# gopi-erabati/Object-Pose-Estimation

Hardware: AMD Instinct MI355X
Metric: ICP iterations/sec (1M scene pts vs 100k model pts) at 1/2/4/8 GPU (higher is better)
Workload: dtype f32

## Files before the change

### object-pose-estimation_amd/csrc/api.hip

```cpp
#include <algorithm>
#include <cfloat>
#include <cmath>
#include <cstring>
#include <limits>
#include <numeric>

#include <chrono>
#include <thread>

#include "ope_internal.hpp"

namespace ope {

void launch_icp_accumulate(hipStream_t, int, int, bool, bool, const CloudView &, const BvhView &, const BvhView &,
                           const IcpState *, double *, int32_t *, float *, uint32_t *, uint32_t *, const uint32_t *,
                           uint32_t *, const uint32_t *, bool, int, double *, const uint32_t *, float *, const uint32_t *, hipEvent_t, hipEvent_t, bool,
                           uint32_t *, uint32_t, float4 *, uint32_t *, uint32_t *, uint32_t, uint32_t, float *);
void plan_heavy(hipStream_t, const uint32_t *, uint32_t, float, float, uint32_t, uint32_t *);
void plan_slots(hipStream_t, const uint32_t *, uint32_t, const uint32_t *, uint32_t *);
int icp_accumulate_blocks_per_cu(bool, bool, bool);
int icp_accumulate_cert_blocks_per_cu(bool, bool, bool);
int chunk_plan(hipStream_t, const uint32_t *, uint32_t *, const uint32_t *, uint32_t *, uint32_t, void *, size_t &);
void fill_iota(hipStream_t, uint32_t *, uint32_t);
hipError_t concat_device(hipStream_t, const CloudView &, const float *, const CloudView &, float *, float[3], float[3], const uint32_t *,
                         const uint32_t *, uint32_t *);
hipError_t build_bvh_device(hipStream_t, const float4 *, const float4 *, size_t, int, const float[3], const float[3], int *, float4 **,
                            float4 **, float4 **, float4 **, bool);
void launch_icp_accumulate_grid(hipStream_t, int, bool, const CloudView &, const BvhView &, const GridView &, const IcpState *, double *, int32_t *,
                                float *, uint32_t *, uint32_t *, const uint32_t *, unsigned char *, const uint32_t *, uint32_t *, const uint32_t *,
                                double *, hipEvent_t, hipEvent_t, bool, uint32_t *, uint32_t, uint32_t *, uint32_t, uint32_t, float4 *, uint32_t *, uint32_t *, float *);
int grid_plan(hipStream_t, bool, const unsigned char *, uint32_t, uint32_t *, uint32_t *, const uint32_t *, uint32_t *, uint32_t *, const uint32_t *,
              uint32_t *, uint32_t, uint32_t, float, float, void *, size_t);
// ... 13 lines not shown
void launch_lm_pos_to_orig(hipStream_t, const BvhView &, int32_t *, uint32_t);
void launch_nn_search(hipStream_t, const CloudView &, const BvhView &, const float *, int32_t *, float *);
void launch_knn_search(hipStream_t, const CloudView &, const BvhView &, const float *, int, int32_t *, float *);
void launch_fitness(hipStream_t, int, const CloudView &, const BvhView &, const float *, double, double *, const uint32_t *);
void launch_seed_hints(hipStream_t, const CloudView &, const BvhView &, const IcpState *, uint32_t *);
void launch_pairs_svd(hipStream_t, const float *, const float *, uint32_t, double *, int, float *);
int comm_allreduce_sums(ope_ctx *ctx, double *d_sums, int count);
bool comm_uses_p2p(const ope_ctx *ctx);
int comm_p2p_exchange_update(ope_ctx *ctx, IcpState *d_state, double *d_sums, int nsums);
int comm_p2p_exchange(ope_ctx *ctx, double *d_sums, int nsums);

static thread_local std::string g_global_err;

constexpr double kGridMaxTreeShare = 0.03, kGridMinTreeShare = 0.015;
constexpr size_t kGridMinQueries = 0;
constexpr float kHeavyLoadFactor = 1.5f;
constexpr float kHeavyMaxChunksPerWave = 1.8f;

int set_err(ope_ctx *ctx, int code, const std::string &msg) {
  if (ctx) ctx->err = msg;
  else g_global_err = msg;
  return code;
}

static inline bool finite3(const float *p) { return std::isfinite(p[0]) && std::isfinite(p[1]) && std::isfinite(p[2]); }

static void colmajor_to_rows(const float *T, float rows[12]) {
  for (int r = 0; r < 3; ++r)
    for (int c = 0; c < 4; ++c) rows[4 * r + c] = T[4 * c + r];
}

// ... 107 lines not shown
  }
  if (ctx->use_grid) {
    const ope_icp_params &p = ctx->run_params;
    const bool nrm = p.use_surface_normal_rej || p.use_self_occluded_rej || p.estimator == OPE_EST_POINT_TO_PLANE_LLS;
    const bool plan_step = !no_plan && nch > 1 && it_done >= 1 && plan_step_after(ctx, it_done);
    if (grid_probe_poll(ctx, it_done) < 0) {
      const int rcs = switch_kernel(ctx, false, it_done, nch);
      if (rcs != OPE_OK) return rcs;
      --ctx->acc_launches;
      return enqueue_accumulate(ctx, atomic_sums);
    }
    if (plan_step) {
      const bool repart = it_done <= 4 || it_done % kPlanPeriod == 0 || it_done == ctx->force_plan_at;
      if (grid_plan(ctx->stream, repart, ctx->d_qclass, (uint32_t)ctx->run_src->n_valid, ctx->d_qorder, ctx->d_work_counter + 8, cost_r,
                    ctx->d_chunk_keys, ctx->d_chunk_cost_sorted, ctx->d_chunk_ids, ctx->d_chunk_order, nch,
                    (uint32_t)ctx->acc_blocks * (kAccBlock / 64), -1.0f , kHeavyLoadFactor, ctx->d_part_tmp, ctx->part_tmp_bytes) != 0)
        return set_err(ctx, OPE_EHIP, "grid plan step failed");
      ctx->plan_valid = true;
      if (it_done == 1 || it_done >= 8) {
        const int rcp = grid_probe_issue(ctx);
        if (rcp != OPE_OK) return rcp;
      }
    }
    const bool timed = ctx->prof_enabled && ctx->prof_used < ctx->prof_events.size() / 2;
    const bool certify = ctx->cert_run && ctx->cert_seen;
    ctx->launch_blocks = certify ? std::min(ctx->acc_blocks, ctx->acc_blocks_cert) : ctx->acc_blocks;
    ++ctx->kernel_launches[OPE_KERNEL_GRID];
    launch_icp_accumulate_grid(ctx->stream, ctx->launch_blocks, nrm, ctx->run_src->view(), ctx->run_tgt->view(), ctx->run_tgt->grid, ctx->d_state,
                               ctx->d_partials, ctx->d_corr_match, ctx->d_corr_d2, ctx->d_hint, ctx->d_ghint, ctx->d_qorder, ctx->d_qclass,
                               ctx->plan_valid ? ctx->d_chunk_order : nullptr, cost_w, ctx->d_work_counter + 8,
                               atomic_sums ? sums_ptr(ctx) : nullptr, timed ? ctx->prof_events[2 * ctx->prof_used] : nullptr,
// ... 8 lines not shown
    if (rcs != OPE_OK) return rcs;
    --ctx->acc_launches;
    return enqueue_accumulate(ctx, atomic_sums);
  }
  if (ctx->plan_pending) {
    OPE_HIP(ctx, hipStreamWaitEvent(ctx->stream, ctx->ev_plan_done, 0));
    ctx->plan_cur ^= 1;
    ctx->plan_cur_slots = ctx->plan_pending_slots;
    ctx->plan_valid = true;
    ctx->plan_pending = false;
  }
  const bool plan_step = !no_plan && nch > 1 && it_done >= 1 && plan_step_after(ctx, it_done);
  if (plan_step) {
    const float chunks_per_wave = (float)nch / (float)(ctx->n_cu * 4 * kAccWavesPerSimd);
    const float heavy_factor = chunks_per_wave > kHeavyMaxChunksPerWave ? 0.0f : std::min(7.0f, std::max(2.0f, 1.2f + 1.5f * chunks_per_wave));
    const float load_factor = chunks_per_wave > kHeavyMaxChunksPerWave ? kHeavyLoadFactor : 0.0f;
    hipStream_t ps = ctx->plan_stream;
    const int nxt = ctx->plan_cur ^ 1;
    OPE_HIP(ctx, hipEventRecord(ctx->ev_acc_done, ctx->stream));
    OPE_HIP(ctx, hipStreamWaitEvent(ps, ctx->ev_acc_done, 0));
    if (ctx->grid_auto && it_done >= 8) {
      const int rcp = grid_probe_issue(ctx, ps);
      if (rcp != OPE_OK) return rcp;
    }
    size_t tb = ctx->plan_tmp_bytes;
    if (chunk_plan(ps, cost_r, ctx->d_plan_sorted[nxt], ctx->d_chunk_ids, ctx->d_plan_order[nxt], nch, ctx->d_plan_tmp, tb) != 0)
      return set_err(ctx, OPE_EHIP, "chunk plan sort failed");
    uint32_t *out = ctx->d_plan_out + 8 * nxt;
    plan_heavy(ps, ctx->d_plan_sorted[nxt], nch, heavy_factor, load_factor, (uint32_t)ctx->acc_blocks * (kAccBlock / 64), out);
    const bool slots = ctx->run_params.corr_mode == OPE_CORR_NEAREST && !ctx->run_params.use_reciprocal;
    if (slots) plan_slots(ps, ctx->d_plan_sorted[nxt], nch, out, ctx->d_plan_slots[nxt]);
// ... 7 lines not shown
  const bool timed = ctx->prof_enabled && ctx->prof_used < ctx->prof_events.size() / 2;
  const bool recip = p.use_reciprocal != 0;
  const uint32_t packet_min = (uint32_t)ctx->n_cu * 4u * (uint32_t)kAccWavesPerSimd;
  const bool packet = p.tree_walk == OPE_WALK_PACKET ? (ctx->run_tgt->d_axis2 != nullptr && p.corr_mode == OPE_CORR_NEAREST && !recip)
                      : p.tree_walk == OPE_WALK_LANE ? false : nch > packet_min;
  ++ctx->kernel_launches[p.corr_mode != OPE_CORR_NEAREST ? OPE_KERNEL_KNN : (packet && !recip) ? OPE_KERNEL_TREE_PACKET : OPE_KERNEL_TREE_LANE];
  const bool certify = ctx->cert_run && ctx->cert_seen && p.corr_mode == OPE_CORR_NEAREST && !recip;
  const int blocks = certify ? std::min(ctx->acc_blocks, ctx->acc_blocks_cert) : ctx->acc_blocks;
  ctx->launch_blocks = blocks;
  launch_icp_accumulate(ctx->stream, blocks, p.corr_mode, nrm, recip, ctx->run_src->view(), ctx->run_tgt->view(),
                        recip ? ctx->run_src_index->view() : ctx->run_tgt->view(), ctx->d_state, ctx->d_partials, ctx->d_corr_match, ctx->d_corr_d2, ctx->d_work_counter, ctx->d_hint,
                        ctx->plan_valid ? ctx->d_plan_order[ctx->plan_cur] : nullptr, cost_w, ctx->d_work_counter + 8, packet, p.k_normal_shooting, atomic_sums ? sums_ptr(ctx) : nullptr,
                        (ctx->plan_valid && ctx->plan_cur_slots) ? ctx->d_plan_slots[ctx->plan_cur] : nullptr,
                        p.corr_mode == OPE_CORR_NORMAL_SHOOTING ? ctx->d_knn_rk : nullptr, ctx->d_plan_out + 8 * ctx->plan_cur,
                        timed ? ctx->prof_events[2 * ctx->prof_used] : nullptr, timed ? ctx->prof_events[2 * ctx->prof_used + 1] : nullptr,
                        ctx->measuring_flag, ctx->chain_on ? chain_ptr(ctx) : nullptr, ctx->chain_seq, certify ? ctx->d_cert_q : nullptr, ctx->d_cert_pos, ctx->d_pace, ++ctx->launch_no, ctx->wait_ticks, ctx->d_cert_l);
  if (timed) ++ctx->prof_used;
  return OPE_OK;
}

__global__ __launch_bounds__(256) void prime_stream_kernel(uint32_t *word, int n) {
  volatile uint32_t buf[64];
  for (int i = 0; i < 64; ++i) buf[i] = (uint32_t)(i * n) + threadIdx.x;
  uint32_t acc = 0u;
  for (int i = 0; i < 64; ++i) acc += buf[(i * 7 + n) & 63];
  if (blockIdx.x == 0 && threadIdx.x == 0) *word = acc | 1u;
}

}

using namespace ope;
// ... 20 lines not shown
  {
    hipDeviceProp_t prop;
    if (hipGetDeviceProperties(&prop, device_ordinal) == hipSuccess && prop.multiProcessorCount > 0) ctx->n_cu = prop.multiProcessorCount;
    int nx = 0;
    if (hipDeviceGetAttribute(&nx, hipDeviceAttributeNumberOfXccs, device_ordinal) == hipSuccess && nx > 0 && nx <= 64) ctx->n_xcd = nx;
  }
  if (hipSetDevice(device_ordinal) != hipSuccess || hipStreamCreate(&ctx->own_stream) != hipSuccess) {
    delete ctx;
    return set_err(nullptr, OPE_EHIP, "hipSetDevice/hipStreamCreate failed");
  }
  ctx->stream = ctx->own_stream;
  if (const char *e = getenv("ROCPROF_COUNTER_COLLECTION"); e != nullptr && *e != 0 && *e != '0') ctx->chain_broken = true;
  if (hipMalloc(&ctx->d_state, sizeof(IcpState)) != hipSuccess ||
      hipMalloc(&ctx->d_partials, sizeof(double) * kNumSumsMax * kAccMaxBlocks) != hipSuccess ||
      hipMalloc((void **)&ctx->d_work_counter, 256) != hipSuccess ||
      hipMalloc((void **)&ctx->d_lm_stats, sizeof(double) * 96) != hipSuccess ||
      hipMalloc((void **)&ctx->d_plan_out, 64) != hipSuccess || hipMemset(ctx->d_plan_out, 0, 64) != hipSuccess ||
      hipStreamCreateWithFlags(&ctx->plan_stream, hipStreamNonBlocking) != hipSuccess ||
      hipStreamCreateWithFlags(&ctx->upd_stream, hipStreamNonBlocking) != hipSuccess ||
      hipEventCreateWithFlags(&ctx->ev_chain_s, hipEventDisableTiming) != hipSuccess ||
      hipEventCreateWithFlags(&ctx->ev_chain_u, hipEventDisableTiming) != hipSuccess ||
      hipEventCreateWithFlags(&ctx->ev_acc_done, hipEventDisableTiming) != hipSuccess ||
      hipEventCreateWithFlags(&ctx->ev_plan_done, hipEventDisableTiming) != hipSuccess ||
      hipHostMalloc((void **)&ctx->h_pace, 64, hipHostMallocMapped) != hipSuccess ||
      hipHostGetDevicePointer((void **)&ctx->d_pace, ctx->h_pace, 0) != hipSuccess ||
      hipHostMalloc((void **)&ctx->h_state, sizeof(IcpState)) != hipSuccess) {
    ope_ctx_destroy(ctx);
    return set_err(nullptr, OPE_ENOMEM, "context allocation failed");
  }
  {
// ... 12 lines not shown
  *out = ctx;
  return OPE_OK;
}

void ope_ctx_destroy(ope_ctx *ctx) {
  if (!ctx) return;
  (void)hipSetDevice(ctx->device);
  ope_comm_destroy(ctx);
  if (ctx->run_src_index) ope_index_free(ctx->run_src_index);
  for (hipEvent_t e : ctx->prof_events) (void)hipEventDestroy(e);
  for (auto &k : ctx->kstamps) { (void)hipEventDestroy(k.e0); (void)hipEventDestroy(k.e1); }
  for (hipEvent_t e : ctx->kevent_pool) (void)hipEventDestroy(e);
  if (ctx->d_state) (void)hipFree(ctx->d_state);
  if (ctx->d_partials) (void)hipFree(ctx->d_partials);
  if (ctx->d_work_counter) (void)hipFree(ctx->d_work_counter);
  if (ctx->d_lm_stats) (void)hipFree(ctx->d_lm_stats);
  if (ctx->d_fixed) (void)hipFree(ctx->d_fixed);
  tmp_release_stream(ctx->stream);
  if (ctx->plan_stream) { (void)hipStreamSynchronize(ctx->plan_stream); (void)hipStreamDestroy(ctx->plan_stream); }
  if (ctx->upd_stream) { (void)hipStreamSynchronize(ctx->upd_stream); (void)hipStreamDestroy(ctx->upd_stream); }
  if (ctx->ev_chain_s) (void)hipEventDestroy(ctx->ev_chain_s);
  if (ctx->ev_chain_u) (void)hipEventDestroy(ctx->ev_chain_u);
  if (ctx->ev_acc_done) (void)hipEventDestroy(ctx->ev_acc_done);
  if (ctx->ev_plan_done) (void)hipEventDestroy(ctx->ev_plan_done);
  for (void *q : {(void *)ctx->d_plan_out, (void *)ctx->d_cost_snap, (void *)ctx->d_plan_sorted[0], (void *)ctx->d_plan_sorted[1], (void *)ctx->d_plan_order[0],
                  (void *)ctx->d_plan_order[1], (void *)ctx->d_plan_slots[0], (void *)ctx->d_plan_slots[1]})
    if (q) (void)hipFree(q);
  if (ctx->d_corr_match) (void)hipFree(ctx->d_corr_match);
  if (ctx->d_corr_d2) (void)hipFree(ctx->d_corr_d2);
  if (ctx->d_hint) (void)hipFree(ctx->d_hint);
// ... 736 lines not shown
  if (ctx->cert_run) {
    OPE_HIP(ctx, hipMemsetAsync(ctx->d_cert_pos, 0, sizeof(uint32_t) * std::max<size_t>(src->n, 1), ctx->stream));
    OPE_HIP(ctx, hipMemsetAsync(ctx->d_corr_d2, 0x7f, sizeof(float) * std::max<size_t>(src->n, 1), ctx->stream));
  }
  if (ctx->run_src_index) { ope_index_free(ctx->run_src_index); ctx->run_src_index = nullptr; }
  if (p.use_reciprocal) {
    int rc = ope_index_build(ctx, src, nullptr, &ctx->run_src_index);
    if (rc != OPE_OK) return rc;
  }
  OPE_HIP(ctx, hipMemcpyAsync(ctx->d_state, h, sizeof *h, hipMemcpyHostToDevice, ctx->stream));
  if (p.corr_mode == OPE_CORR_NORMAL_SHOOTING && p.max_iterations > 1 && src->n_valid > 0)
    launch_seed_hints(ctx->stream, src->view(), tgt->view(), ctx->d_state, ctx->d_hint);
  if (ctx->d_sums_ext)
    OPE_HIP(ctx, hipMemsetAsync(ctx->d_sums_ext, 0, sizeof(double) * (p.estimator == OPE_EST_POINT_TO_PLANE_LLS ? kNumSumsMax : kNumSums), ctx->stream));
  OPE_HIP(ctx, hipMemsetAsync(ctx->d_work_counter, 0, 256, ctx->stream));
  OPE_HIP(ctx, hipMemsetAsync(ctx->d_lm_stats, 0, sizeof(double) * 96, ctx->stream));
  ctx->measuring_flag = false;
  OPE_HIP(ctx, hipMemsetAsync(ctx->d_partials, 0, sizeof(double) * kNumSumsMax * kAccMaxBlocks, ctx->stream));
  OPE_HIP(ctx, hipStreamSynchronize(ctx->stream));
  ctx->h_pace[0] = 0u; ctx->h_pace[1] = 0u;
  ctx->launch_no = 0;
  ctx->pace_off = false;
  ctx->run_src = src;
  ctx->run_tgt = tgt;
  ctx->corr_run_n = src->n;
  ctx->run_params = p;
  ctx->run_active = true;
  ctx->iters_enqueued = 0;
  const int block = (p.corr_mode == OPE_CORR_NEAREST && !p.use_reciprocal) ? kAccBlock : ((p.corr_mode == OPE_CORR_NEAREST) ? kAccBlock : 256);
  ctx->acc_blocks = (int)std::min<size_t>(std::max<size_t>(2 * ((src->n_valid + block - 1) / block), 1), kAccMaxBlocks);
// ... 486 lines not shown
```

### object-pose-estimation_amd/csrc/icp_kernels.hip

```cpp
#include <cstdlib>
#include <hip/hip_ext.h>

#include "bvh_traverse.hpp"
#include "lm_solve.hpp"
#include "icp_update.hpp"

namespace ope {

typedef const __attribute__((address_space(3))) float *lds_cfloat_ptr;
static_assert(kCertCand >= 1 && kCertCand <= 8, "skip certificates: candidates per query");

__device__ __forceinline__ uint32_t chain_load(const uint32_t *p) { return __hip_atomic_load(p, __ATOMIC_RELAXED, __HIP_MEMORY_SCOPE_AGENT); }
__device__ __forceinline__ void chain_store(uint32_t *p, uint32_t v) { __hip_atomic_store(p, v, __ATOMIC_RELAXED, __HIP_MEMORY_SCOPE_AGENT); }
__device__ __forceinline__ void chain_wait_own_memory_ops() { __builtin_amdgcn_s_waitcnt(0); }
__device__ __forceinline__ bool acc_launch_begin(const IcpState *st, uint32_t *chain, uint32_t chain_seq, float *s_const, uint32_t wait_ticks) {
  if (chain == nullptr) return st->done == 0;
  __shared__ uint32_t s_go[2];
  if (threadIdx.x == 0) {
    uint32_t go = 1u;
    const unsigned long long t0 = wall_clock64();
    while ((int32_t)(chain_load(chain + 1) - chain_seq) < 0) {
      if (wall_clock64() - t0 > (unsigned long long)wait_ticks) { go = 0u; atomicOr(chain + 2, 1u); break; }
      __builtin_amdgcn_s_sleep(2);
    }
    s_go[0] = go;
  }
  __syncthreads();
  if (threadIdx.x < 12) s_const[threadIdx.x] = __hip_atomic_load(&st->Ff[threadIdx.x], __ATOMIC_RELAXED, __HIP_MEMORY_SCOPE_AGENT);
  else if (threadIdx.x == 12) s_go[1] = (uint32_t)__hip_atomic_load(&st->done, __ATOMIC_RELAXED, __HIP_MEMORY_SCOPE_AGENT);
  else if (threadIdx.x == 17) s_const[17] = __hip_atomic_load(&st->last_move, __ATOMIC_RELAXED, __HIP_MEMORY_SCOPE_AGENT);
  __syncthreads();
  return s_go[0] != 0u && s_go[1] == 0u;
}
__device__ __forceinline__ void acc_launch_end(uint32_t *chain) {
  if (chain == nullptr) return;
  chain_wait_own_memory_ops();
  __syncthreads();
  if (threadIdx.x == 0) __hip_atomic_fetch_add(chain, 1u, __ATOMIC_RELAXED, __HIP_MEMORY_SCOPE_AGENT);
}

template <bool NRM>
__device__ __forceinline__ void add_query_sums(double *acc, lds_cfloat_ptr cs2, uint32_t lane_id, bool ok, bool p2p, float x, float y, float z,
                                               const float4 t, const float4 tn, float d2) {
    {
      asm volatile("" : "+v"(cs2));
      const float psx = cs2[12], psy = cs2[13], psz = cs2[14];
      const double sx = (double)x - (double)psx, sy = (double)y - (double)psy, sz = (double)z - (double)psz;
      const double tx = (double)t.x - (double)psx, ty = (double)t.y - (double)psy, tz = (double)t.z - (double)psz;
      const double w = ok ? 1.0 : 0.0;
      double term[kNumSums];
      term[0] = w;
      term[1] = w * sx; term[2] = w * sy; term[3] = w * sz;
      term[4] = w * tx; term[5] = w * ty; term[6] = w * tz;
// ... 92 lines not shown
  }
}
__device__ __forceinline__ bool cert_worth_building(float d2_prev, float cert_k, float cert_cap, float last_move) {
  const float dprev = __builtin_amdgcn_sqrtf(d2_prev);
  return fminf(cert_cap, cert_k * __builtin_amdgcn_rcpf(dprev)) >= kCertWorth * last_move;
}

constexpr int kKnnWavesPerSimd = 4;
template <int MODE, bool NRM, bool RECIP = false, bool PACKET = false, int KREG = 20, bool CERT = false>
__global__ __launch_bounds__(MODE == 0 ? kAccBlock : kKnnBlock, (MODE == 0 && !RECIP && !CERT) ? kAccWavesPerSimd : (MODE == 2 ? kKnnWavesPerSimd : 4)) void icp_accumulate_kernel(
    CloudView src, BvhView tgt, BvhView srcix, const IcpState *__restrict__ st, double *__restrict__ partials,
    int32_t *__restrict__ corr_match, float *__restrict__ corr_d2, uint32_t *__restrict__ work_counter,
    uint32_t *__restrict__ hint, const uint32_t *__restrict__ chunk_order, uint32_t *__restrict__ chunk_cost,
    const uint32_t *__restrict__ plan_info, double *__restrict__ S_atomic, const uint32_t *__restrict__ slot_list,
    float *__restrict__ knn_rk, const uint32_t *__restrict__ plan_out, uint32_t measuring_launch, uint32_t *chain_arg, uint32_t chain_seq,
    float4 *__restrict__ cert_q, uint32_t *__restrict__ cert_pos, uint32_t *pace, uint32_t launch_no, uint32_t wait_ticks, float *__restrict__ cert_l) {
  if (pace != nullptr && blockIdx.x == 0 && threadIdx.x == 0) __hip_atomic_store(pace, launch_no, __ATOMIC_RELAXED, __HIP_MEMORY_SCOPE_SYSTEM);
  uint32_t *const chain = (MODE == 0 && !RECIP) ? chain_arg : nullptr;
  static_assert(!CERT || (MODE == 0 && !RECIP), "skip certificates: plain 1-NN only");
  __shared__ __attribute__((aligned(16))) float s_const[20];
  __shared__ uint32_t s_ncert;
  if (!acc_launch_begin(st, chain, chain_seq, s_const, wait_ticks)) return;
  constexpr int BLOCK = (MODE == 0) ? kAccBlock : kKnnBlock;
  constexpr bool OCT_OK = (MODE == 0) && !RECIP;
  __shared__ double s_red[BLOCK / 64][kNumSumsMax];
  __shared__ float s_stk[kMaxDepth + 2][BLOCK];
  float *stk = &s_stk[0][threadIdx.x];
  extern __shared__ unsigned char s_dyn[];

  const double max_d2 = st->max_d2;
  float best0 = INFINITY;
// ... 16 lines not shown
    if (blockIdx.x == 0) atomicAdd(work_counter + 42, 1u);
  }
  if (cert_on) __syncthreads();
  const bool rej_sn = NRM && st->use_surface_normal_rej;
  const bool rej_so = NRM && st->use_self_occluded_rej;
  const bool store_pos = st->estimator == OPE_EST_POINT_TO_PLANE_LM;
  const double thr_sn = st->surface_normal_thr, thr_so = st->self_occluded_thr;
  const double max_dist_unsq = st->max_corr_dist;
  const int kk = st->k_normal_shooting;

  if ((threadIdx.x & 63u) < (uint32_t)kNumSumsMax) s_red[threadIdx.x >> 6][threadIdx.x & 63u] = 0.0;
  const bool p2p = NRM && st->estimator == OPE_EST_POINT_TO_PLANE_LLS;

  const uint32_t lane_id = threadIdx.x & 63u;
  const uint32_t n_waves = gridDim.x * (BLOCK / 64);
  const uint32_t wave_id = blockIdx.x * (BLOCK / 64) + (threadIdx.x >> 6);
  const uint32_t n_chunks = (src.n_valid + 63u) / 64u;
  const bool measuring = chunk_order && measuring_launch != 0u;
  const uint32_t n_heavy = (OCT_OK && chunk_order && !measuring) ? min(plan_out[0], n_chunks) : 0u;
  const bool listed = OCT_OK && slot_list != nullptr && chunk_order != nullptr && !measuring && n_heavy > 0u;
  const uint32_t n_alone = !chunk_order ? 0u
                           : listed   ? min(plan_out[7], n_waves / 2u)
                                      : min(min(plan_out[5] + (measuring ? min(plan_out[0], n_chunks) : 0u), n_chunks - n_heavy), n_waves / 2u);
  const uint32_t n_snake = listed ? (n_chunks + 7u * n_heavy - n_alone) : (8u * n_heavy + (n_chunks - n_heavy - n_alone));
  const uint32_t snake_waves = n_waves - n_alone;
  for (uint32_t round = 0;; ++round) {
    bool oct = false;
    uint32_t ord, sub = 0;
    uint32_t slot;
    if (wave_id < n_alone) {
      if (round > 0) break;
      slot = wave_id;
      ord = n_heavy + wave_id;
    } else {
      if (round * snake_waves >= n_snake) break;
      const uint32_t w = wave_id - n_alone;
      slot = round * snake_waves + ((round & 1u) ? (snake_waves - 1u - w) : w);
      if (slot >= n_snake) continue;
      oct = slot < 8u * n_heavy;
      ord = oct ? (slot >> 3) : (n_heavy + n_alone + (slot - 8u * n_heavy));
      sub = slot & 7u;
      slot += n_alone;
    }
    if (listed) {
      const uint32_t e = slot_list[slot];
      oct = (e >> 31) != 0u;
      sub = (e >> 28) & 7u;
      ord = e & 0x0fffffffu;
    }
    const uint32_t chunk = chunk_order ? chunk_order[ord] : ord;
    const uint32_t base = chunk * 64u;
    const unsigned long long t_begin = __builtin_amdgcn_s_memtime();
    const uint32_t i = oct ? (base + sub * 8u + (lane_id >> 3)) : (base + lane_id);
    const bool active = i < src.n_valid;
    const bool owner = active && (!oct || (lane_id & 7u) == 0u);
    lds_cfloat_ptr cst = (lds_cfloat_ptr)s_const;
    asm volatile("" : "+v"(cst));
    float F[12];
#pragma unroll
    for (int k = 0; k < 12; ++k) F[k] = cst[k];
    const float4 s = src.xyzw[active ? i : base];
    const float x = xform_row(F + 0, s.x, s.y, s.z);
    const float y = xform_row(F + 4, s.x, s.y, s.z);
// ... 6 lines not shown
      nz = rot_row(F + 8, n4.x, n4.y, n4.z);
    }
    bool ok;
    float d2;
    uint32_t pos = 0;
    int match = -1;
    if constexpr (CERT) {
      const float best_init = active ? cst[15] : -INFINITY;
      const size_t cstride = src.n;
      bool need = active, stuck = false, has_cert = false;
      float c_best = INFINITY;
      uint32_t c_pos = 0u;
      if (active) need = !cert_check(tgt, cert_q, cert_l, cert_pos, cstride, i, x, y, z, best_init, cst[17], c_best, c_pos, stuck, has_cert);
      const bool build = need && !stuck && owner && cert_worth_building(corr_d2[i], cst[18], cst[19], cst[17]);
      const uint32_t h = need ? hint[i] : 0u;
      const bool fast = need && !build && !(oct && __shfl((int)build, (int)(lane_id & ~7u), 64) != 0);
      NearestVisitor v{fast ? best_init : -INFINITY, kNoPos, 0};
      const unsigned long long fmask = __ballot(fast);
      if (fmask != 0ull) {
        if (oct) {
          if (fast) bvh_traverse_oct(tgt, x, y, z, v, &s_stk[0][threadIdx.x & ~7u], BLOCK, h);
        } else if (__popcll(fmask) <= 8) {
          const uint32_t r = lane_id >> 3;
          const bool serve = r < (uint32_t)__popcll(fmask);
          unsigned long long mm = fmask;
          for (uint32_t k = 0; k < r && mm != 0ull; ++k) mm &= mm - 1ull;
          const int from = mm != 0ull ? (int)__builtin_ctzll(mm) : 0;
          const float gx = __shfl(x, from, 64), gy = __shfl(y, from, 64), gz = __shfl(z, from, 64);
          const uint32_t gh = (uint32_t)__shfl((int)h, from, 64);
          NearestVisitor gv{serve ? cst[15] : -INFINITY, kNoPos, 0};
// ... 11 lines not shown
      uint32_t r_pos = fast ? v.pos : c_pos, r_leaf = fast ? v.leaf : h;
      if (__ballot(build) != 0ull) cert_build(tgt, cert_q, cert_l, cert_pos, cstride, i, x, y, z, best_init, h, stk, BLOCK, build, build, r_best, r_pos, r_leaf);
      {
        const uint32_t nc = (uint32_t)__popcll(__ballot(owner && !need));
        if (lane_id == 0 && nc != 0u) atomicAdd(&s_ncert, nc);
      }
      if (owner && r_leaf != h) hint[i] = r_leaf;
      const bool found = active && r_pos != kNoPos;
      pos = found ? r_pos : 0;
      ok = found && !((double)r_best > max_d2);
      d2 = found ? r_best : INFINITY;
      match = found ? (store_pos ? (int)pos : __float_as_int(tgt.pts[pos].w)) : -1;
    } else if constexpr (MODE == 0) {
      NearestVisitor v{active ? cst[15] : -INFINITY, kNoPos, 0};
      const uint32_t h = active ? hint[i] : 0u;
      if (OCT_OK && oct) {
        if (active) bvh_traverse_oct(tgt, x, y, z, v, &s_stk[0][threadIdx.x & ~7u], BLOCK, h);
      } else {
        const bool done = PACKET && bvh_traverse_packet(tgt, x, y, z, active, v, h, stk, BLOCK);
        if (!done && active) bvh_traverse_deferred(tgt, x, y, z, v, stk, BLOCK, h, min(8, kMaxDepth + 1 - tgt.depth));
      }
      if (owner && v.leaf != h) hint[i] = v.leaf;
      const bool found = active && v.pos != kNoPos;
      ok = found && !((double)v.best > max_d2);
      d2 = found ? v.best : INFINITY;
      pos = found ? v.pos : 0;
      match = found ? (store_pos ? (int)pos : __float_as_int(tgt.pts[pos].w)) : -1;
      if (RECIP) {
        float G[12];
#pragma unroll
// ... 7 lines not shown
      }
    } else if constexpr (MODE == 2) {
      constexpr int K = KREG;
      KnnRegVisitor<K> v;
      float bound0 = INFINITY;
      if (knn_rk != nullptr && active && st->have_prev) {
        const float rk = knn_rk[i];
        if (rk < 3.0e38f) {
          const float ox = xform_row(st->Fprev + 0, s.x, s.y, s.z), oy = xform_row(st->Fprev + 4, s.x, s.y, s.z), oz = xform_row(st->Fprev + 8, s.x, s.y, s.z);
          const float delta = sqrtf(sq_dist3(x - ox, y - oy, z - oz));
          const float b = sqrtf(rk) * 1.00001f + delta * 1.00001f + 1e-6f * (fabsf(x) + fabsf(y) + fabsf(z)) + 1e-30f;
          bound0 = b * b * 1.00001f;
        }
      }
      const uint32_t h0 = active ? hint[i] : 0u;
      bool todo = active;
      for (;;) {
        if (todo) {
          v.init(true, bound0);
          bvh_traverse(tgt, x, y, z, v, stk, BLOCK, h0);
        }
        const bool retry = todo && bound0 < 3.0e38f && v.count < K;
        if (__ballot(retry) == 0ull) break;
        todo = retry;
        bound0 = INFINITY;
      }
      if (!active) v.init(false);
      if (active) {
        hint[i] = v.leaf;
        if (knn_rk != nullptr) knn_rk[i] = v.count >= K ? v.d[K - 1] : INFINITY;
// ... 4 lines not shown
#pragma unroll
      for (int j = 0; j < K; ++j) {
        if (j < v.count && j < kk) {
          const float4 p = tgt.pts[v.p[j]];
          const double vx = (double)__fsub_rn(p.x, x), vy = (double)__fsub_rn(p.y, y), vz = (double)__fsub_rn(p.z, z);
          const double cx = (double)ny * vz - (double)nz * vy;
          const double cy = (double)nz * vx - (double)nx * vz;
          const double cz = (double)nx * vy - (double)ny * vx;
          const double dist = cx * cx + cy * cy + cz * cz;
          if (dist < min_dist) { min_dist = dist; d2 = v.d[j]; pos = v.p[j]; }
        }
      }
      ok = active && v.count > 0 && !(min_dist > max_dist_unsq);
      match = v.count > 0 ? (store_pos ? (int)pos : __float_as_int(tgt.pts[pos].w)) : -1;
    } else {
      float *ld = reinterpret_cast<float *>(s_dyn) + threadIdx.x;
      uint32_t *lp = reinterpret_cast<uint32_t *>(s_dyn + sizeof(float) * BLOCK * kKnnMaxK) + threadIdx.x;
      KnnVisitor v{ld, lp, BLOCK, kk, 0, active ? INFINITY : -INFINITY};
      bvh_traverse(tgt, x, y, z, v, stk, BLOCK);
      double min_dist = 1.79769313486231570815e308;
      int min_j = 0;
      for (int j = 0; j < v.count; ++j) {
        const float4 p = tgt.pts[lp[j * BLOCK]];
        const double vx = (double)__fsub_rn(p.x, x), vy = (double)__fsub_rn(p.y, y), vz = (double)__fsub_rn(p.z, z);
        const double cx = (double)ny * vz - (double)nz * vy;
        const double cy = (double)nz * vx - (double)nx * vz;
        const double cz = (double)nx * vy - (double)ny * vx;
        const double dist = cx * cx + cy * cy + cz * cz;
        if (dist < min_dist) { min_dist = dist; min_j = j; }
      }
// ... 8 lines not shown
      ok = (double)score > thr_sn;
    }
    if (NRM && ok && rej_so) {
      const double sl = sqrt((double)__fadd_rn(__fadd_rn(__fmul_rn(x, x), __fmul_rn(y, y)), __fmul_rn(z, z)));
      const double score = (double)nx * (-(double)x / sl) + (double)ny * (-(double)y / sl) + (double)nz * (-(double)z / sl);
      ok = score > thr_so;
    }
    ok = ok && owner;
    if (owner) {
      __builtin_nontemporal_store(ok ? match : -1, corr_match + i);
      __builtin_nontemporal_store(d2, corr_d2 + i);
    }
    add_query_sums<NRM>(s_red[threadIdx.x >> 6], (lds_cfloat_ptr)s_const, lane_id, ok, p2p, x, y, z, tgt.pts[ok ? pos : 0],
                        (NRM && p2p) ? tgt.nrm[ok ? pos : 0] : make_float4(0.f, 0.f, 0.f, 0.f), d2);
    if (lane_id == 0 && !oct) chunk_cost[chunk] = (uint32_t)((__builtin_amdgcn_s_memtime() - t_begin) >> 4);
  }

  __syncthreads();
  if (threadIdx.x < (p2p ? kNumSumsMax : kNumSums)) {
    double v = 0.0;
#pragma unroll
    for (int w = 0; w < BLOCK / 64; ++w) v += s_red[w][threadIdx.x];
    if (S_atomic != nullptr) unsafeAtomicAdd(S_atomic + threadIdx.x, v);
    else partials[threadIdx.x * kAccMaxBlocks + blockIdx.x] = v;
  }
  if (CERT && threadIdx.x == 64 && s_ncert != 0u)
    atomicAdd(reinterpret_cast<unsigned long long *>(work_counter + 40), (unsigned long long)s_ncert);
  acc_launch_end(chain);
}

// ... 640 lines not shown
  const int lane = threadIdx.x & 63, wave = threadIdx.x >> 6;
  if (lane == 0) { s_red[wave][0] = sum; s_red[wave][1] = cnt; }
  __syncthreads();
  if (threadIdx.x < 2) {
    partials[2 * blockIdx.x + threadIdx.x] =
        s_red[0][threadIdx.x] + s_red[1][threadIdx.x] + s_red[2][threadIdx.x] + s_red[3][threadIdx.x];
  }
}

void launch_icp_accumulate(hipStream_t stream, int nblocks, int mode, bool nrm, bool recip, const CloudView &src,
                           const BvhView &tgt, const BvhView &srcix, const IcpState *st, double *partials,
                           int32_t *corr_match, float *corr_d2, uint32_t *work_counter, uint32_t *hint,
                           const uint32_t *chunk_order, uint32_t *chunk_cost, const uint32_t *plan_info, bool packet,
                           int k_normal_shooting, double *S_atomic, const uint32_t *slot_list, float *knn_rk, const uint32_t *plan_out,
                           hipEvent_t e0, hipEvent_t e1, bool measuring, uint32_t *chain, uint32_t chain_seq, float4 *cert_q, uint32_t *cert_pos,
                           uint32_t *pace, uint32_t launch_no, uint32_t wait_ticks, float *cert_l) {
  const uint32_t mflag = measuring ? 1u : 0u;
#define OPE_KLAUNCH(KERNEL, BLK, LDS)                                                                                         \
  do {                                                                                                                        \
    if (e0 != nullptr)                                                                                                        \
      hipExtLaunchKernelGGL(KERNEL, dim3(nblocks), dim3(BLK), LDS, stream, e0, e1, 0, src, tgt, srcix, st, partials, corr_match, \
                            corr_d2, work_counter, hint, chunk_order, chunk_cost, plan_info, S_atomic, slot_list, knn_rk, plan_out, mflag, chain, chain_seq, cert_q, cert_pos, pace, launch_no, wait_ticks, cert_l); \
    else                                                                                                                      \
      hipLaunchKernelGGL(KERNEL, dim3(nblocks), dim3(BLK), LDS, stream, src, tgt, srcix, st, partials, corr_match, corr_d2,   \
                         work_counter, hint, chunk_order, chunk_cost, plan_info, S_atomic, slot_list, knn_rk, plan_out, mflag, chain, chain_seq, cert_q, cert_pos, pace, launch_no, wait_ticks, cert_l); \
  } while (0)
#define OPE_LAUNCH_ACC(M, N, R, BLK, LDS) OPE_KLAUNCH((icp_accumulate_kernel<M, N, R>), BLK, LDS)
  const bool certify = cert_q != nullptr && mode == 0 && !recip;
  if (mode == 0 && !recip && packet) {
    if (certify) { if (nrm) OPE_KLAUNCH((icp_accumulate_kernel<0, true, false, true, 20, true>), kAccBlock, 0); else OPE_KLAUNCH((icp_accumulate_kernel<0, false, false, true, 20, true>), kAccBlock, 0); }
    else if (nrm) OPE_KLAUNCH((icp_accumulate_kernel<0, true, false, true>), kAccBlock, 0);
    else OPE_KLAUNCH((icp_accumulate_kernel<0, false, false, true>), kAccBlock, 0);
    return;
  }
  if (mode == 0) {
    if (recip) { if (nrm) OPE_LAUNCH_ACC(0, true, true, kAccBlock, 0); else OPE_LAUNCH_ACC(0, false, true, kAccBlock, 0); }
    else if (certify) { if (nrm) OPE_KLAUNCH((icp_accumulate_kernel<0, true, false, false, 20, true>), kAccBlock, 0); else OPE_KLAUNCH((icp_accumulate_kernel<0, false, false, false, 20, true>), kAccBlock, 0); }
    else       { if (nrm) OPE_LAUNCH_ACC(0, true, false, kAccBlock, 0); else OPE_LAUNCH_ACC(0, false, false, kAccBlock, 0); }
  } else {
#define OPE_LAUNCH_NS(KR) OPE_KLAUNCH((icp_accumulate_kernel<2, true, false, false, KR>), kKnnBlock, 0)
// ... 128 lines not shown
```

### object-pose-estimation_amd/csrc/ope_internal.hpp

```cpp
#pragma once

#include <hip/hip_runtime.h>

#include <algorithm>
#include <cstdint>
#include <memory>
#include <mutex>
#include <string>
#include <utility>
#include <cstdio>
#include <cstdlib>
#include <cstring>
#include <vector>

#include "../../include/ope.h"

namespace ope {

constexpr int kNodeFloats = 12;
constexpr int kMaxDepth = 20;
constexpr size_t kPtsPad = 8;

struct BvhView {
  const float4 *nodes;
// ... 63 lines not shown
constexpr int kP2pSlotWords = 2 * kP2pMaxSums;
constexpr size_t kP2pBufferBytes = sizeof(unsigned long long) * 2 * kP2pMaxRanks * kP2pSlotWords;
struct P2pView {
  unsigned long long *buf[kP2pMaxRanks];
  int nranks, rank;
};

constexpr float kOctSlotShare = 0.42f;
constexpr float kCertWorth = 24.0f;
constexpr int kCertCand = 5;
constexpr int kNumSums = 17;
constexpr int kNumSumsMax = 44;
constexpr int kAccBlock = 512;
constexpr int kAccWavesPerSimd = 6;
constexpr int kAccMaxBlocks = 1024;

}

template <class T>
struct default_init_allocator : std::allocator<T> {
  template <class U> struct rebind { using other = default_init_allocator<U>; };
  using std::allocator<T>::allocator;
  template <class U, class... Args> void construct(U *p, Args &&...args) {
    if constexpr (sizeof...(Args) == 0) ::new (static_cast<void *>(p)) U;
    else ::new (static_cast<void *>(p)) U(std::forward<Args>(args)...);
  }
};

struct ope_ctx {
  int device = -1;
// ... 1 lines not shown
  int n_xcd = 8;
  uint32_t wait_ticks = 200000000u;
  hipStream_t own_stream = nullptr;
  hipStream_t stream = nullptr;
  std::string err;

  ope::IcpState *d_state = nullptr;
  double *d_partials = nullptr;
  double *d_lm_stats = nullptr;
  uint32_t *d_work_counter = nullptr;
  int32_t *d_corr_match = nullptr;
  float *d_corr_d2 = nullptr;
  uint32_t *d_chunk_cost = nullptr, *d_chunk_cost_sorted = nullptr, *d_chunk_ids = nullptr, *d_chunk_order = nullptr;
  uint32_t *d_slot_list = nullptr;
  bool slot_list_valid = false;
  void *d_plan_tmp = nullptr;
  size_t plan_tmp_bytes = 0, chunk_cap = 0;
  bool plan_valid = false;
  hipStream_t plan_stream = nullptr;
  hipEvent_t ev_acc_done = nullptr, ev_plan_done = nullptr;
  uint32_t *d_cost_snap = nullptr;
  uint32_t *d_plan_sorted[2] = {nullptr, nullptr}, *d_plan_order[2] = {nullptr, nullptr}, *d_plan_slots[2] = {nullptr, nullptr};
  uint32_t *d_plan_out = nullptr;
  int plan_cur = 0;
  bool plan_pending = false, plan_pending_slots = false, plan_cur_slots = false;
  int acc_launches = 0;
  hipStream_t upd_stream = nullptr;
  hipEvent_t ev_chain_s = nullptr, ev_chain_u = nullptr;
  bool chained = false;
  bool chain_on = false;
// ... 337 lines not shown
```

Measured before the change: 16250.

## Replace static snake chunk schedule with striped atomic work dealing in accumulate kernel

```diff
diff --git a/object-pose-estimation_amd/csrc/api.hip b/object-pose-estimation_amd/csrc/api.hip
--- a/object-pose-estimation_amd/csrc/api.hip
+++ b/object-pose-estimation_amd/csrc/api.hip
@@ -15,7 +15,7 @@
 void launch_icp_accumulate(hipStream_t, int, int, bool, bool, const CloudView &, const BvhView &, const BvhView &,
                            const IcpState *, double *, int32_t *, float *, uint32_t *, uint32_t *, const uint32_t *,
                            uint32_t *, const uint32_t *, bool, int, double *, const uint32_t *, float *, const uint32_t *, hipEvent_t, hipEvent_t, bool,
-                           uint32_t *, uint32_t, float4 *, uint32_t *, uint32_t *, uint32_t, uint32_t, float *);
+                           uint32_t *, uint32_t, float4 *, uint32_t *, uint32_t *, uint32_t, uint32_t, float *, uint32_t *, uint32_t);
 void plan_heavy(hipStream_t, const uint32_t *, uint32_t, float, float, uint32_t, uint32_t *);
 void plan_slots(hipStream_t, const uint32_t *, uint32_t, const uint32_t *, uint32_t *);
 int icp_accumulate_blocks_per_cu(bool, bool, bool);
@@ -59,7 +59,8 @@
 
 constexpr double kGridMaxTreeShare = 0.03, kGridMinTreeShare = 0.015;
 constexpr size_t kGridMinQueries = 0;
-constexpr float kHeavyLoadFactor = 1.5f;
+constexpr float kHeavyLoadFactor = 1.0f;
+constexpr float kHeavyLoadFactorStatic = 1.5f;
 constexpr float kHeavyMaxChunksPerWave = 1.8f;
 
 int set_err(ope_ctx *ctx, int code, const std::string &msg) {
@@ -197,7 +198,7 @@
       const bool repart = it_done <= 4 || it_done % kPlanPeriod == 0 || it_done == ctx->force_plan_at;
       if (grid_plan(ctx->stream, repart, ctx->d_qclass, (uint32_t)ctx->run_src->n_valid, ctx->d_qorder, ctx->d_work_counter + 8, cost_r,
                     ctx->d_chunk_keys, ctx->d_chunk_cost_sorted, ctx->d_chunk_ids, ctx->d_chunk_order, nch,
-                    (uint32_t)ctx->acc_blocks * (kAccBlock / 64), -1.0f , kHeavyLoadFactor, ctx->d_part_tmp, ctx->part_tmp_bytes) != 0)
+                    (uint32_t)ctx->acc_blocks * (kAccBlock / 64), -1.0f , kHeavyLoadFactorStatic, ctx->d_part_tmp, ctx->part_tmp_bytes) != 0)
         return set_err(ctx, OPE_EHIP, "grid plan step failed");
       ctx->plan_valid = true;
       if (it_done == 1 || it_done >= 8) {
@@ -236,7 +237,8 @@
   if (plan_step) {
     const float chunks_per_wave = (float)nch / (float)(ctx->n_cu * 4 * kAccWavesPerSimd);
     const float heavy_factor = chunks_per_wave > kHeavyMaxChunksPerWave ? 0.0f : std::min(7.0f, std::max(2.0f, 1.2f + 1.5f * chunks_per_wave));
-    const float load_factor = chunks_per_wave > kHeavyMaxChunksPerWave ? kHeavyLoadFactor : 0.0f;
+    const bool static_deal = ctx->cert_run && ctx->cert_seen && ctx->run_params.corr_mode == OPE_CORR_NEAREST && !ctx->run_params.use_reciprocal;
+    const float load_factor = chunks_per_wave > kHeavyMaxChunksPerWave ? (static_deal ? kHeavyLoadFactorStatic : kHeavyLoadFactor) : 0.0f;
     hipStream_t ps = ctx->plan_stream;
     const int nxt = ctx->plan_cur ^ 1;
     OPE_HIP(ctx, hipEventRecord(ctx->ev_acc_done, ctx->stream));
@@ -274,7 +276,9 @@
                         (ctx->plan_valid && ctx->plan_cur_slots) ? ctx->d_plan_slots[ctx->plan_cur] : nullptr,
                         p.corr_mode == OPE_CORR_NORMAL_SHOOTING ? ctx->d_knn_rk : nullptr, ctx->d_plan_out + 8 * ctx->plan_cur,
                         timed ? ctx->prof_events[2 * ctx->prof_used] : nullptr, timed ? ctx->prof_events[2 * ctx->prof_used + 1] : nullptr,
-                        ctx->measuring_flag, ctx->chain_on ? chain_ptr(ctx) : nullptr, ctx->chain_seq, certify ? ctx->d_cert_q : nullptr, ctx->d_cert_pos, ctx->d_pace, ++ctx->launch_no, ctx->wait_ticks, ctx->d_cert_l);
+                        ctx->measuring_flag, ctx->chain_on ? chain_ptr(ctx) : nullptr, ctx->chain_seq, certify ? ctx->d_cert_q : nullptr, ctx->d_cert_pos, ctx->d_pace, ++ctx->launch_no, ctx->wait_ticks, ctx->d_cert_l,
+                        ctx->d_deal, ctx->deal_parity);
+  ctx->deal_parity ^= 1u;
   if (timed) ++ctx->prof_used;
   return OPE_OK;
 }
@@ -325,6 +329,7 @@
   if (hipMalloc(&ctx->d_state, sizeof(IcpState)) != hipSuccess ||
       hipMalloc(&ctx->d_partials, sizeof(double) * kNumSumsMax * kAccMaxBlocks) != hipSuccess ||
       hipMalloc((void **)&ctx->d_work_counter, 256) != hipSuccess ||
+      hipMalloc((void **)&ctx->d_deal, kDealBytes) != hipSuccess || hipMemset(ctx->d_deal, 0, kDealBytes) != hipSuccess ||
       hipMalloc((void **)&ctx->d_lm_stats, sizeof(double) * 96) != hipSuccess ||
       hipMalloc((void **)&ctx->d_plan_out, 64) != hipSuccess || hipMemset(ctx->d_plan_out, 0, 64) != hipSuccess ||
       hipStreamCreateWithFlags(&ctx->plan_stream, hipStreamNonBlocking) != hipSuccess ||
@@ -367,6 +372,7 @@
   if (ctx->d_state) (void)hipFree(ctx->d_state);
   if (ctx->d_partials) (void)hipFree(ctx->d_partials);
   if (ctx->d_work_counter) (void)hipFree(ctx->d_work_counter);
+  if (ctx->d_deal) (void)hipFree(ctx->d_deal);
   if (ctx->d_lm_stats) (void)hipFree(ctx->d_lm_stats);
   if (ctx->d_fixed) (void)hipFree(ctx->d_fixed);
   tmp_release_stream(ctx->stream);
@@ -1133,6 +1139,8 @@
   if (ctx->d_sums_ext)
     OPE_HIP(ctx, hipMemsetAsync(ctx->d_sums_ext, 0, sizeof(double) * (p.estimator == OPE_EST_POINT_TO_PLANE_LLS ? kNumSumsMax : kNumSums), ctx->stream));
   OPE_HIP(ctx, hipMemsetAsync(ctx->d_work_counter, 0, 256, ctx->stream));
+  OPE_HIP(ctx, hipMemsetAsync(ctx->d_deal, 0, kDealBytes, ctx->stream));
+  ctx->deal_parity = 0;
   OPE_HIP(ctx, hipMemsetAsync(ctx->d_lm_stats, 0, sizeof(double) * 96, ctx->stream));
   ctx->measuring_flag = false;
   OPE_HIP(ctx, hipMemsetAsync(ctx->d_partials, 0, sizeof(double) * kNumSumsMax * kAccMaxBlocks, ctx->stream));
diff --git a/object-pose-estimation_amd/csrc/icp_kernels.hip b/object-pose-estimation_amd/csrc/icp_kernels.hip
--- a/object-pose-estimation_amd/csrc/icp_kernels.hip
+++ b/object-pose-estimation_amd/csrc/icp_kernels.hip
@@ -37,6 +37,21 @@
   chain_wait_own_memory_ops();
   __syncthreads();
   if (threadIdx.x == 0) __hip_atomic_fetch_add(chain, 1u, __ATOMIC_RELAXED, __HIP_MEMORY_SCOPE_AGENT);
+}
+
+__device__ __forceinline__ uint32_t deal_pop(uint32_t *counters, uint32_t stripe, uint32_t lane_id) {
+  uint32_t k = 0u;
+  if (lane_id == 0u) k = __hip_atomic_fetch_add(counters + stripe * kDealLineWords, 1u, __ATOMIC_RELAXED, __HIP_MEMORY_SCOPE_AGENT);
+  return k;
+}
+constexpr uint32_t kDealNone = 0xffffffffu;
+__device__ __forceinline__ uint32_t deal_next(uint32_t k, uint32_t stripe, uint32_t n_stripes, uint32_t n_waves, uint32_t n_slots) {
+  const uint32_t slot = n_waves + stripe + k * n_stripes;
+  return slot < n_slots ? slot : kDealNone;
+}
+__device__ __forceinline__ void deal_clear_other_set(uint32_t *deal, uint32_t parity) {
+  if (blockIdx.x == 0 && threadIdx.x < kDealStripes)
+    __hip_atomic_store(deal + (size_t)(parity ^ 1u) * kDealStripes * kDealLineWords + threadIdx.x * kDealLineWords, 0u, __ATOMIC_RELAXED, __HIP_MEMORY_SCOPE_AGENT);
 }
 
 template <bool NRM>
@@ -159,7 +174,9 @@
     uint32_t *__restrict__ hint, const uint32_t *__restrict__ chunk_order, uint32_t *__restrict__ chunk_cost,
     const uint32_t *__restrict__ plan_info, double *__restrict__ S_atomic, const uint32_t *__restrict__ slot_list,
     float *__restrict__ knn_rk, const uint32_t *__restrict__ plan_out, uint32_t measuring_launch, uint32_t *chain_arg, uint32_t chain_seq,
-    float4 *__restrict__ cert_q, uint32_t *__restrict__ cert_pos, uint32_t *pace, uint32_t launch_no, uint32_t wait_ticks, float *__restrict__ cert_l) {
+    float4 *__restrict__ cert_q, uint32_t *__restrict__ cert_pos, uint32_t *pace, uint32_t launch_no, uint32_t wait_ticks, float *__restrict__ cert_l,
+    uint32_t *deal, uint32_t deal_parity) {
+  deal_clear_other_set(deal, deal_parity);
   if (pace != nullptr && blockIdx.x == 0 && threadIdx.x == 0) __hip_atomic_store(pace, launch_no, __ATOMIC_RELAXED, __HIP_MEMORY_SCOPE_SYSTEM);
   uint32_t *const chain = (MODE == 0 && !RECIP) ? chain_arg : nullptr;
   static_assert(!CERT || (MODE == 0 && !RECIP), "skip certificates: plain 1-NN only");
@@ -206,39 +223,42 @@
 
   const uint32_t lane_id = threadIdx.x & 63u;
   const uint32_t n_waves = gridDim.x * (BLOCK / 64);
-  const uint32_t wave_id = blockIdx.x * (BLOCK / 64) + (threadIdx.x >> 6);
+  const uint32_t wave_id = (uint32_t)__builtin_amdgcn_readfirstlane((int)(blockIdx.x * (BLOCK / 64) + (threadIdx.x >> 6)));
   const uint32_t n_chunks = (src.n_valid + 63u) / 64u;
   const bool measuring = chunk_order && measuring_launch != 0u;
   const uint32_t n_heavy = (OCT_OK && chunk_order && !measuring) ? min(plan_out[0], n_chunks) : 0u;
   const bool listed = OCT_OK && slot_list != nullptr && chunk_order != nullptr && !measuring && n_heavy > 0u;
-  const uint32_t n_alone = !chunk_order ? 0u
-                           : listed   ? min(plan_out[7], n_waves / 2u)
-                                      : min(min(plan_out[5] + (measuring ? min(plan_out[0], n_chunks) : 0u), n_chunks - n_heavy), n_waves / 2u);
-  const uint32_t n_snake = listed ? (n_chunks + 7u * n_heavy - n_alone) : (8u * n_heavy + (n_chunks - n_heavy - n_alone));
-  const uint32_t snake_waves = n_waves - n_alone;
-  for (uint32_t round = 0;; ++round) {
-    bool oct = false;
-    uint32_t ord, sub = 0;
-    uint32_t slot;
-    if (wave_id < n_alone) {
-      if (round > 0) break;
-      slot = wave_id;
-      ord = n_heavy + wave_id;
-    } else {
-      if (round * snake_waves >= n_snake) break;
-      const uint32_t w = wave_id - n_alone;
-      slot = round * snake_waves + ((round & 1u) ? (snake_waves - 1u - w) : w);
-      if (slot >= n_snake) continue;
-      oct = slot < 8u * n_heavy;
-      ord = oct ? (slot >> 3) : (n_heavy + n_alone + (slot - 8u * n_heavy));
-      sub = slot & 7u;
-      slot += n_alone;
-    }
+  const uint32_t n_slots = n_chunks + 7u * n_heavy;
+  const bool dealt = chunk_order != nullptr && !CERT;
+  uint32_t *const deal_set = deal + (size_t)deal_parity * kDealStripes * kDealLineWords;
+  const uint32_t n_stripes = min(kDealStripes, n_waves);
+  const uint32_t stripe = wave_id % n_stripes;
+  const uint32_t n_alone = (dealt || !chunk_order) ? 0u
+                           : listed             ? min(plan_out[7], n_waves / 2u)
+                                                : min(min(plan_out[5] + (measuring ? min(plan_out[0], n_chunks) : 0u), n_chunks - n_heavy), n_waves / 2u);
+  const uint32_t n_snake = n_slots - n_alone, snake_waves = n_waves - n_alone;
+  auto static_slot = [&](uint32_t r) -> uint32_t {
+    if (wave_id < n_alone) return r == 0u ? (listed ? wave_id : 8u * n_heavy + wave_id) : kDealNone;
+    const uint32_t w = wave_id - n_alone;
+    const uint32_t sn = r * snake_waves + ((r & 1u) ? (snake_waves - 1u - w) : w);
+    if (sn >= n_snake) return kDealNone;
+    return (listed || sn >= 8u * n_heavy) ? sn + n_alone : sn;
+  };
+  uint32_t round = 0u;
+  uint32_t slot = static_slot(0u);
+  while (slot != kDealNone) {
+    uint32_t ticket_v = 0u;
+    bool oct;
+    uint32_t ord, sub;
     if (listed) {
       const uint32_t e = slot_list[slot];
       oct = (e >> 31) != 0u;
       sub = (e >> 28) & 7u;
       ord = e & 0x0fffffffu;
+    } else {
+      oct = slot < 8u * n_heavy;
+      ord = oct ? (slot >> 3) : (n_heavy + (slot - 8u * n_heavy));
+      sub = slot & 7u;
     }
     const uint32_t chunk = chunk_order ? chunk_order[ord] : ord;
     const uint32_t base = chunk * 64u;
@@ -275,6 +295,7 @@
       if (active) need = !cert_check(tgt, cert_q, cert_l, cert_pos, cstride, i, x, y, z, best_init, cst[17], c_best, c_pos, stuck, has_cert);
       const bool build = need && !stuck && owner && cert_worth_building(corr_d2[i], cst[18], cst[19], cst[17]);
       const uint32_t h = need ? hint[i] : 0u;
+      if (dealt) ticket_v = deal_pop(deal_set, stripe, lane_id);
       const bool fast = need && !build && !(oct && __shfl((int)build, (int)(lane_id & ~7u), 64) != 0);
       NearestVisitor v{fast ? best_init : -INFINITY, kNoPos, 0};
       const unsigned long long fmask = __ballot(fast);
@@ -316,6 +337,7 @@
     } else if constexpr (MODE == 0) {
       NearestVisitor v{active ? cst[15] : -INFINITY, kNoPos, 0};
       const uint32_t h = active ? hint[i] : 0u;
+      if (dealt) ticket_v = deal_pop(deal_set, stripe, lane_id);
       if (OCT_OK && oct) {
         if (active) bvh_traverse_oct(tgt, x, y, z, v, &s_stk[0][threadIdx.x & ~7u], BLOCK, h);
       } else {
@@ -353,6 +375,7 @@
         }
       }
       const uint32_t h0 = active ? hint[i] : 0u;
+      if (dealt) ticket_v = deal_pop(deal_set, stripe, lane_id);
       bool todo = active;
       for (;;) {
         if (todo) {
@@ -387,6 +410,7 @@
       ok = active && v.count > 0 && !(min_dist > max_dist_unsq);
       match = v.count > 0 ? (store_pos ? (int)pos : __float_as_int(tgt.pts[pos].w)) : -1;
     } else {
+      if (dealt) ticket_v = deal_pop(deal_set, stripe, lane_id);
       float *ld = reinterpret_cast<float *>(s_dyn) + threadIdx.x;
       uint32_t *lp = reinterpret_cast<uint32_t *>(s_dyn + sizeof(float) * BLOCK * kKnnMaxK) + threadIdx.x;
       KnnVisitor v{ld, lp, BLOCK, kk, 0, active ? INFINITY : -INFINITY};
@@ -425,6 +449,11 @@
     add_query_sums<NRM>(s_red[threadIdx.x >> 6], (lds_cfloat_ptr)s_const, lane_id, ok, p2p, x, y, z, tgt.pts[ok ? pos : 0],
                         (NRM && p2p) ? tgt.nrm[ok ? pos : 0] : make_float4(0.f, 0.f, 0.f, 0.f), d2);
     if (lane_id == 0 && !oct) chunk_cost[chunk] = (uint32_t)((__builtin_amdgcn_s_memtime() - t_begin) >> 4);
+    if (dealt) {
+      slot = deal_next((uint32_t)__builtin_amdgcn_readfirstlane((int)ticket_v), stripe, n_stripes, n_waves, n_slots);
+    } else {
+      slot = static_slot(++round);
+    }
   }
 
   __syncthreads();
@@ -1095,16 +1124,16 @@
                            const uint32_t *chunk_order, uint32_t *chunk_cost, const uint32_t *plan_info, bool packet,
                            int k_normal_shooting, double *S_atomic, const uint32_t *slot_list, float *knn_rk, const uint32_t *plan_out,
                            hipEvent_t e0, hipEvent_t e1, bool measuring, uint32_t *chain, uint32_t chain_seq, float4 *cert_q, uint32_t *cert_pos,
-                           uint32_t *pace, uint32_t launch_no, uint32_t wait_ticks, float *cert_l) {
+                           uint32_t *pace, uint32_t launch_no, uint32_t wait_ticks, float *cert_l, uint32_t *deal, uint32_t deal_parity) {
   const uint32_t mflag = measuring ? 1u : 0u;
 #define OPE_KLAUNCH(KERNEL, BLK, LDS)                                                                                         \
   do {                                                                                                                        \
     if (e0 != nullptr)                                                                                                        \
       hipExtLaunchKernelGGL(KERNEL, dim3(nblocks), dim3(BLK), LDS, stream, e0, e1, 0, src, tgt, srcix, st, partials, corr_match, \
-                            corr_d2, work_counter, hint, chunk_order, chunk_cost, plan_info, S_atomic, slot_list, knn_rk, plan_out, mflag, chain, chain_seq, cert_q, cert_pos, pace, launch_no, wait_ticks, cert_l); \
+                            corr_d2, work_counter, hint, chunk_order, chunk_cost, plan_info, S_atomic, slot_list, knn_rk, plan_out, mflag, chain, chain_seq, cert_q, cert_pos, pace, launch_no, wait_ticks, cert_l, deal, deal_parity); \
     else                                                                                                                      \
       hipLaunchKernelGGL(KERNEL, dim3(nblocks), dim3(BLK), LDS, stream, src, tgt, srcix, st, partials, corr_match, corr_d2,   \
-                         work_counter, hint, chunk_order, chunk_cost, plan_info, S_atomic, slot_list, knn_rk, plan_out, mflag, chain, chain_seq, cert_q, cert_pos, pace, launch_no, wait_ticks, cert_l); \
+                         work_counter, hint, chunk_order, chunk_cost, plan_info, S_atomic, slot_list, knn_rk, plan_out, mflag, chain, chain_seq, cert_q, cert_pos, pace, launch_no, wait_ticks, cert_l, deal, deal_parity); \
   } while (0)
 #define OPE_LAUNCH_ACC(M, N, R, BLK, LDS) OPE_KLAUNCH((icp_accumulate_kernel<M, N, R>), BLK, LDS)
   const bool certify = cert_q != nullptr && mode == 0 && !recip;
diff --git a/object-pose-estimation_amd/csrc/ope_internal.hpp b/object-pose-estimation_amd/csrc/ope_internal.hpp
--- a/object-pose-estimation_amd/csrc/ope_internal.hpp
+++ b/object-pose-estimation_amd/csrc/ope_internal.hpp
@@ -101,6 +101,9 @@
 constexpr int kAccBlock = 512;
 constexpr int kAccWavesPerSimd = 6;
 constexpr int kAccMaxBlocks = 1024;
+constexpr uint32_t kDealStripes = 64;
+constexpr uint32_t kDealLineWords = 32;
+constexpr size_t kDealBytes = sizeof(uint32_t) * 2 * kDealStripes * kDealLineWords;
 
 }
 
@@ -132,6 +135,8 @@
   uint32_t *d_chunk_cost = nullptr, *d_chunk_cost_sorted = nullptr, *d_chunk_ids = nullptr, *d_chunk_order = nullptr;
   uint32_t *d_slot_list = nullptr;
   bool slot_list_valid = false;
+  uint32_t *d_deal = nullptr;
+  uint32_t deal_parity = 0;
   void *d_plan_tmp = nullptr;
   size_t plan_tmp_bytes = 0, chunk_cap = 0;
   bool plan_valid = false;
```

After: 16560, median of 6. 1.9% higher.
